# yshen47/SGAM_NeurIPS22

Hardware: AMD Instinct MI355X
Metric: generated RGB-D frames/sec (256x256, GoogleEarth) (higher is better)
Workload: dtype f32; 1 GPU; GoogleEarth-Infinite 256x256 inference loop (BASELINE configs[2]): forward-splat warp (N<=3) + VQGAN encode/quantise(4096)/decode + frame feedback, in-HBM frame store; frames_per_gpu=1105, scenes=1, parallelism=scene-parallel x1, launch=hip-graph replay of the VQGAN forward, f32_products=exact hi/lo fp16 split on the fp16 matrix cores, fp32 accumulate

## Files before the change

include/sgam_hip.h:

```cpp
#ifndef SGAM_HIP_H
#define SGAM_HIP_H

#include <stdint.h>

#ifdef __cplusplus
extern "C" {
#endif

#define SGAM_OK 0
#define SGAM_EINVAL (-1)
#define SGAM_EALIGN (-2)
#define SGAM_EWORKSPACE (-3)

int sgam_abi_version(void);
const char *sgam_build_info(void);
const char *sgam_build_commit(void);
const char *sgam_build_digest(void);

int sgam_prof_enable(int32_t on);
int sgam_prof_mark_empty(void *stream);
int32_t sgam_prof_count(void);
int sgam_prof_get(int32_t i, const char **kernel, const char **where, float *ms, double *flops, double *bytes);
int sgam_prof_get_shape(int32_t i, int32_t *mnks);

// ... 19 lines not shown
                            float *out, void *workspace, int64_t workspace_bytes, void *stream);

int sgam_pack_conv_weight(const float *w_oihw, float *w_packed, int32_t Cout, int32_t Cin, int32_t KH,
                          int32_t KW, int32_t Cout_pad, int32_t Cin_pad, void *stream);

int sgam_f32x_set_range_flag(int32_t *device_flag);
int64_t sgam_conv2d_f32x_workspace_bytes(const sgam_conv_desc *d);
int sgam_conv2d_f32x_plan(const sgam_conv_desc *d, int32_t *bm, int32_t *bn, int32_t *ksplit);
int sgam_conv2d_nhwc_f32x(const sgam_conv_desc *d, const float *x, float a_scale, const void *w_planes,
                          float w_scale, const float *bias, const float *residual, float *out, void *workspace,
                          int64_t workspace_bytes, void *stream);
int sgam_pack_conv_weight_f32x(const float *w_oihw, void *w_planes, float w_scale, int32_t Cout, int32_t Cin,
                               int32_t KH, int32_t KW, int32_t Cout_pad, int32_t Cin_pad, void *stream);
int32_t sgam_conv2d_f32x_stats_chunks(const sgam_conv_desc *d);
int32_t sgam_conv2d_f32x_stats_mode(const sgam_conv_desc *d);
int sgam_conv2d_stats_nhwc_f32x(const sgam_conv_desc *d, const float *x, float a_scale, const void *w_planes,
                                float w_scale, const float *bias, const float *residual, float *out,
                                double *gn_partial, void *workspace, int64_t workspace_bytes, void *stream);
int sgam_groupnorm_from_partials_f32(const float *x, const double *partial, int32_t nchunk, const float *gamma,
                                     const float *beta, float *y, int32_t B, int32_t HW, int32_t C, int32_t groups,
                                     float eps, int32_t fuse_swish, void *workspace, int64_t workspace_bytes, void *stream);
int32_t sgam_conv2d_f32x_gn_fusable(const sgam_conv_desc *d);
int32_t sgam_conv2d_f32x_uses_halo(const sgam_conv_desc *d);
int sgam_conv2d_gn_nhwc_f32x(const sgam_conv_desc *d, const float *x, const float *gn_mean_rstd, const float *gn_gamma,
                             const float *gn_beta, int32_t gn_swish, const void *w_planes, float w_scale, const float *bias,
                             const float *residual, float *out, double *gn_partial, void *workspace, int64_t workspace_bytes,
                             void *stream);
int32_t sgam_conv2d_f32x_gn_foldable(const sgam_conv_desc *d, int32_t chunks_in);
int sgam_conv2d_gnp_nhwc_f32x(const sgam_conv_desc *d, const float *x, const double *gn_partial_in, int32_t chunks_in, float eps,
                              const float *gn_gamma, const float *gn_beta, int32_t gn_swish, const void *w_planes, float w_scale,
                              const float *bias, const float *residual, float *out, double *gn_partial, void *workspace,
                              int64_t workspace_bytes, void *stream);
int sgam_groupnorm_stats_from_partials_f32(const double *partial, int32_t nchunk, float *mean_rstd, int32_t B, int32_t HW,
                                           int32_t C, int32_t groups, float eps, void *stream);
int sgam_groupnorm_meanrstd_nhwc_f32(const float *x, float *mean_rstd, int32_t B, int32_t HW, int32_t C, int32_t groups,
                                     float eps, void *workspace, int64_t workspace_bytes, void *stream);
int sgam_split_rows_f32x(const float *x, void *planes, float scale, int32_t N, int32_t K, int32_t ld, void *stream);

int64_t sgam_conv2d_h16_workspace_bytes(const sgam_conv_desc *d);
int sgam_conv2d_h16_plan(const sgam_conv_desc *d, int32_t *bm, int32_t *bn, int32_t *ksplit);
int sgam_conv2d_nhwc_h16(const sgam_conv_desc *d, int32_t ht, const void *x, const void *w_packed,
                         const float *bias, const void *residual, void *out, int32_t out_f32, void *workspace,
                         int64_t workspace_bytes, void *stream);
int32_t sgam_conv2d_h16_generic_stats_chunks(const sgam_conv_desc *d);
int sgam_conv2d_stats_nhwc_h16(const sgam_conv_desc *d, int32_t ht, const void *x, const void *w_packed, const float *bias,
                               const void *residual, void *out, int32_t out_f32, double *gn_partial, void *workspace,
// ... 295 lines not shown
```

sgam_neurips22_amd/_lib.py:

```python
import ctypes
import os

_PKG = os.path.dirname(os.path.abspath(__file__))
LIB_PATH = os.environ.get("SGAM_HIP_LIB") or os.path.join(_PKG, "lib", "libsgam_hip.so")

c_i32, c_i64, c_f32, c_vp = ctypes.c_int32, ctypes.c_int64, ctypes.c_float, ctypes.c_void_p


class ConvDesc(ctypes.Structure):
    _fields_ = [(n, c_i32) for n in (
        "B", "Hi", "Wi", "Cin", "Ho", "Wo", "N", "KH", "KW", "stride", "pad_t", "pad_l", "upsample2x",
        "lda", "ldb", "ldc", "ldr", "n_valid", "bias_per_row", "plan_bm", "plan_bn", "plan_ksplit")]


class TsdfGrid(ctypes.Structure):
    _fields_ = [("voxel_length", c_f32), ("sdf_trunc", c_f32), ("unit_base", c_i32 * 3), ("unit_dims", c_i32 * 3)]


class TsdfSrc(ctypes.Structure):
    _fields_ = [("depth", c_vp), ("rgb_u8", c_vp), ("cam2world", c_f32 * 16), ("world2cam", c_f32 * 16)]


class TsdfScene(ctypes.Structure):
    _fields_ = [("unit_table", c_vp), ("unit_stamp", c_vp), ("counters", c_vp), ("brick_list", c_vp), ("brick_tsdf", c_vp),
# ... 14 lines not shown
                              ctypes.POINTER(c_f32), ctypes.POINTER(ctypes.c_double), ctypes.POINTER(ctypes.c_double)]),
    "sgam_prof_get_shape": (c_i32, [c_i32, ctypes.POINTER(c_i32)]),
    "sgam_conv2d_workspace_bytes": (c_i64, [ctypes.POINTER(ConvDesc)]),
    "sgam_conv2d_plan": (c_i32, [ctypes.POINTER(ConvDesc), ctypes.POINTER(c_i32), ctypes.POINTER(c_i32),
                                 ctypes.POINTER(c_i32)]),
    "sgam_conv2d_nhwc_f32": (c_i32, [ctypes.POINTER(ConvDesc), c_vp, c_vp, c_vp, c_vp, c_vp, c_vp, c_i64, c_vp]),
    "sgam_conv2d_gn_nhwc_f32": (c_i32, [ctypes.POINTER(ConvDesc), c_vp, c_vp, c_i32, c_vp, c_vp, c_vp, c_vp, c_vp, c_i64,
                                        c_vp]),
    "sgam_pack_conv_weight": (c_i32, [c_vp, c_vp, c_i32, c_i32, c_i32, c_i32, c_i32, c_i32, c_vp]),
    "sgam_f32x_set_range_flag": (c_i32, [c_vp]),
    "sgam_conv2d_f32x_workspace_bytes": (c_i64, [ctypes.POINTER(ConvDesc)]),
    "sgam_conv2d_f32x_plan": (c_i32, [ctypes.POINTER(ConvDesc), ctypes.POINTER(c_i32), ctypes.POINTER(c_i32),
                                      ctypes.POINTER(c_i32)]),
    "sgam_conv2d_nhwc_f32x": (c_i32, [ctypes.POINTER(ConvDesc), c_vp, c_f32, c_vp, c_f32, c_vp, c_vp, c_vp, c_vp, c_i64,
                                      c_vp]),
    "sgam_conv2d_f32x_stats_chunks": (c_i32, [ctypes.POINTER(ConvDesc)]),
    "sgam_conv2d_f32x_stats_mode": (c_i32, [ctypes.POINTER(ConvDesc)]),
    "sgam_conv2d_stats_nhwc_f32x": (c_i32, [ctypes.POINTER(ConvDesc), c_vp, c_f32, c_vp, c_f32, c_vp, c_vp, c_vp, c_vp, c_vp,
                                            c_i64, c_vp]),
    "sgam_groupnorm_from_partials_f32": (c_i32, [c_vp, c_vp, c_i32, c_vp, c_vp, c_vp, c_i32, c_i32, c_i32, c_i32, c_f32,
                                                 c_i32, c_vp, c_i64, c_vp]),
    "sgam_conv2d_f32x_gn_fusable": (c_i32, [ctypes.POINTER(ConvDesc)]),
    "sgam_conv2d_f32x_uses_halo": (c_i32, [ctypes.POINTER(ConvDesc)]),
    "sgam_conv2d_gn_nhwc_f32x": (c_i32, [ctypes.POINTER(ConvDesc), c_vp, c_vp, c_vp, c_vp, c_i32, c_vp, c_f32, c_vp, c_vp,
                                         c_vp, c_vp, c_vp, c_i64, c_vp]),
    "sgam_conv2d_f32x_gn_foldable": (c_i32, [ctypes.POINTER(ConvDesc), c_i32]),
    "sgam_conv2d_gnp_nhwc_f32x": (c_i32, [ctypes.POINTER(ConvDesc), c_vp, c_vp, c_i32, c_f32, c_vp, c_vp, c_i32, c_vp, c_f32, c_vp,
                                          c_vp, c_vp, c_vp, c_vp, c_i64, c_vp]),
    "sgam_groupnorm_stats_from_partials_f32": (c_i32, [c_vp, c_i32, c_vp, c_i32, c_i32, c_i32, c_i32, c_f32, c_vp]),
    "sgam_groupnorm_meanrstd_nhwc_f32": (c_i32, [c_vp, c_vp, c_i32, c_i32, c_i32, c_i32, c_f32, c_vp, c_i64, c_vp]),
    "sgam_tsdf_integrate_srcs_f32": (c_i32, [ctypes.POINTER(TsdfGrid), ctypes.POINTER(TsdfSrc), c_i32, c_i32, c_i32, c_f32, c_f32, c_f32,
                                             c_f32, c_f32, c_i32, c_vp, c_vp, c_vp, c_vp, c_i32, c_vp, c_vp, c_i32, c_vp, c_vp, c_vp]),
    "sgam_tsdf_integrate_scenes_f32": (c_i32, [ctypes.POINTER(TsdfGrid), c_vp, c_vp, c_i32, c_i32, c_i32, c_i32, c_f32, c_f32, c_f32, c_f32,
                                               c_f32, c_i32, c_i32, c_vp, c_vp]),
    "sgam_tsdf_raycast_scenes_f32": (c_i32, [ctypes.POINTER(TsdfGrid), c_vp, c_vp, c_i32, c_i32, c_i32, c_f32, c_f32, c_f32, c_f32, c_f32,
                                             c_f32, c_vp, c_vp, c_vp]),
    "sgam_tsdf_ray_mult_f32": (c_i32, [c_i32, c_i32, c_f32, c_f32, c_f32, c_f32, c_vp, c_vp]),
    "sgam_tsdf_raycast_depth_f32": (c_i32, [ctypes.POINTER(TsdfGrid), c_i32, c_i32, c_f32, c_f32, c_f32, c_f32, c_vp, c_f32,
                                            c_f32, c_vp, c_vp, c_vp, c_vp, c_vp, c_vp]),
    "sgam_tsdf_extract_points_f32": (c_i32, [ctypes.POINTER(TsdfGrid), c_vp, c_vp, c_vp, c_vp, c_i64, c_vp, c_vp, c_vp, c_vp, c_vp]),
    "sgam_tsdf_mesh_workspace_bytes": (c_i64, [ctypes.POINTER(TsdfGrid), c_i32]),
    "sgam_tsdf_extract_mesh_f32": (c_i32, [ctypes.POINTER(TsdfGrid), c_vp, c_vp, c_vp, c_vp, c_i32, c_vp, c_i32, c_i32, c_f32, c_f32, c_f32,
                                           c_f32, c_f32, c_f32, c_vp, c_vp, c_vp, c_i64, c_vp, c_i64, c_vp, c_vp, c_i64, c_vp]),
    "sgam_mesh_render_depth_f32": (c_i32, [c_vp, c_i64, c_vp, c_i64, c_vp, c_i32, c_i32, c_f32, c_f32, c_f32, c_f32, c_vp, c_f32, c_f32,
                                           c_vp, c_vp]),
    "sgam_gemm_gn_f32x_fits": (c_i32, [c_i32, c_i32, c_i32, c_i32]),
# ... 183 lines not shown
```

sgam_neurips22_amd/csrc/conv_f32x.hip:

```cpp
#include <type_traits>

#include "sgam_common.h"

namespace {

constexpr int XGN_MAXC = 1024;

typedef unsigned int u32x4 __attribute__((ext_vector_type(4)));
typedef unsigned int u32x2 __attribute__((ext_vector_type(2)));
typedef _Float16 f16x8 __attribute__((ext_vector_type(8)));

struct XParams {
    const float *x, *bias, *res;
    const unsigned short *w;
    float *out, *ws;
    int B, Hi, Wi, Cin, Ho, Wo, N, KH, KW, stride, pad_t, pad_l, ups;
    int lda, ldb, ldc, ldr, n_valid, bias_per_row;
    int M, ksplit, iters_total, iters_per_split;
    int gx, gy, xcd_swizzle;
    unsigned x_bytes, w_plane_bytes;
    const float *gn_stats, *gn_gamma, *gn_beta;
    int gn_swish;
    const double *gn_partial_in;
    double gn_inv_n;
// ... 704 lines not shown
        if (s1 - s0 >= 2) {
            slab(s0, I2{}, I0{});
            slab(s0 + 1, I3{}, I3{});
        } else if (s0 < s1) {
            slab(s0, I3{}, I0{});
        }
    } else if (s0 < s1) {
        int sl = s0;
        for (; sl + 2 < s1; sl += 2) {
            slab(sl, I1{}, I0{});
            slab(sl + 1, I1{}, I3{});
        }
        slab(s1 - 2, I2{}, I0{});
        slab(s1 - 1, I3{}, I3{});
    }
    __syncthreads();

    xepilogue<BM, BN, WGM_>(p, acc, reinterpret_cast<float *>(smem), wave, lane, bx, bz, n0, [&](int row) {
        return (b * p.Ho + ty0 + (row >> TWS)) * p.Wo + tx0 + (row & (TW - 1));
    });
}


__global__ __launch_bounds__(256) void splitk_reduce_f32x_kernel(const XParams p) {
    const int64_t q = (int64_t)blockIdx.x * blockDim.x + threadIdx.x;
    const int nq = p.N / 4;
    const bool live = q < (int64_t)p.M * nq;
    const int m = live ? (int)(q / nq) : 0;
    const int n = live ? (int)(q - (int64_t)m * nq) * 4 : 0;
    float gs = 0.f, gss = 0.f;
    if (live) {
        const float *w0 = p.ws + (int64_t)m * p.N + n;
        const int64_t zs = (int64_t)p.M * p.N;
        float bv[4], rv[4];
#pragma unroll
        for (int e = 0; e < 4; ++e) {
            const bool ok = n + e < p.n_valid;
            bv[e] = (ok && p.bias) ? (p.bias_per_row ? p.bias[m] : p.bias[n + e]) : 0.f;
            rv[e] = (ok && p.res) ? p.res[(int64_t)m * p.ldr + n + e] : 0.f;
        }
        f32x4 s = *reinterpret_cast<const f32x4 *>(w0);
        int z = 1;
        for (; z + 4 <= p.ksplit; z += 4) {
            const f32x4 a = *reinterpret_cast<const f32x4 *>(w0 + z * zs), b = *reinterpret_cast<const f32x4 *>(w0 + (z + 1) * zs);
            const f32x4 c = *reinterpret_cast<const f32x4 *>(w0 + (z + 2) * zs), d = *reinterpret_cast<const f32x4 *>(w0 + (z + 3) * zs);
            s += a;
// ... 99 lines not shown
}

__device__ __forceinline__ int64_t frag_index(int64_t n, int64_t k, int64_t slabs_per_row) {
    const int64_t slab = k >> 5, kin = k & 31;
    const int64_t piece = (((kin >> 4) * 2) + ((kin >> 3) & 1)) * 32 + (n & 31);
    return (((n >> 5) * slabs_per_row + slab) * 256 + piece) * 8 + (kin & 7);
}

__global__ void pack_weight_f32x_kernel(const float *w, unsigned short *o, int Cout, int Cin, int KH, int KW, int Cout_pad,
                                        int Cin_pad, float scale) {
    const int64_t i = (int64_t)blockIdx.x * blockDim.x + threadIdx.x;
    const int taps = KH * KW;
    const int64_t total = (int64_t)Cout_pad * taps * Cin_pad;
    if (i >= total) return;
    const int c = (int)(i % Cin_pad);
    const int t = (int)((i / Cin_pad) % taps);
    const int n = (int)(i / ((int64_t)Cin_pad * taps));
    float v = 0.f;
    if (n < Cout && c < Cin) v = w[((int64_t)n * Cin + c) * taps + t] * scale;
    const _Float16 h = (_Float16)v;
    const _Float16 l = (_Float16)(v - (float)h);
    const int64_t k = (int64_t)t * Cin_pad + c;
    const int64_t q = frag_index(n, k, (int64_t)taps * Cin_pad / 32);
    o[q] = __builtin_bit_cast(unsigned short, h);
    o[q + 2 * 2 * 32 * 8] = __builtin_bit_cast(unsigned short, l);
}

__global__ void split_rows_f32x_kernel(const float *x, unsigned short *o, int N, int Np, int K, int Kp, int ld, float scale) {
    const int64_t i = (int64_t)blockIdx.x * blockDim.x + threadIdx.x;
    const int64_t total = (int64_t)Np * Kp;
    if (i >= total) return;
    const int n = (int)(i / Kp), k = (int)(i - (int64_t)n * Kp);
    const float v = (k < K && n < N) ? x[(int64_t)n * ld + k] * scale : 0.f;
    const _Float16 h = (_Float16)v;
    const _Float16 l = (_Float16)(v - (float)h);
    const int64_t q = frag_index(n, k, Kp / 32);
    o[q] = __builtin_bit_cast(unsigned short, h);
    o[q + 2 * 2 * 32 * 8] = __builtin_bit_cast(unsigned short, l);
}

struct XPlan {
    int bm, bn, ksplit, iters_total, iters_per_split;
};

static bool halo_shape(const sgam_conv_desc *d, int bm, int bn) {
    const bool tile_ok = (bm == 128 && bn == 128 && d->Wo % 16 == 0) || (bm == 64 && bn == 128 && d->Wo % 8 == 0) ||
// ... 30 lines not shown
    pl.iters_per_split = (pl.iters_total + ks - 1) / ks;
    if (halo_shape(d, pl.bm, pl.bn)) pl.iters_per_split = (pl.iters_per_split + 8) / 9 * 9;
    pl.ksplit = (pl.iters_total + pl.iters_per_split - 1) / pl.iters_per_split;
    return pl;
}

int xvalidate(const sgam_conv_desc *d) {
    if (!d) return SGAM_EINVAL;
    if (d->B <= 0 || d->Hi <= 0 || d->Wi <= 0 || d->Ho <= 0 || d->Wo <= 0 || d->N <= 0) return SGAM_EINVAL;
    if (d->Cin <= 0 || d->Cin % 8 != 0 || d->N % 4 != 0) return SGAM_EINVAL;
    if (d->KH <= 0 || d->KW <= 0 || d->stride <= 0) return SGAM_EINVAL;
    if (d->lda < d->Cin || d->lda % 4 != 0) return SGAM_EALIGN;
    if (d->ldb < d->KH * d->KW * d->Cin || d->ldb % 32 != 0) return SGAM_EALIGN;
    if (d->KH * d->KW > 1 && d->Cin % 32 != 0) return SGAM_EALIGN;
    if (d->n_valid <= 0 || d->n_valid > d->N || d->ldc < d->n_valid) return SGAM_EINVAL;
    if (d->n_valid % 4 != 0 || d->ldc % 4 != 0 || d->ldr % 4 != 0) return SGAM_EALIGN;
    if (d->plan_bm != 0 || d->plan_bn != 0) {
        const bool ok = (d->plan_bm == 128 && d->plan_bn == 128) || (d->plan_bm == 64 && d->plan_bn == 128) ||
                        (d->plan_bm == 128 && d->plan_bn == 32 && d->N == 32) ||
                        (d->plan_bm == 64 && d->plan_bn == 64);
        if (!ok || (d->plan_bn == 128 && d->N % 128 != 0)) return SGAM_EINVAL;
    }
    if (d->plan_ksplit < 0 || d->plan_ksplit > 64) return SGAM_EINVAL;
    return SGAM_OK;
}

}

extern "C" int64_t sgam_conv2d_f32x_workspace_bytes(const sgam_conv_desc *d) {
    if (xvalidate(d) != SGAM_OK) return -1;
    const XPlan pl = make_xplan(d);
    if (pl.ksplit <= 1) return 0;
    return (int64_t)pl.ksplit * d->B * d->Ho * d->Wo * d->N * (int64_t)sizeof(float);
}

extern "C" int sgam_conv2d_f32x_plan(const sgam_conv_desc *d, int32_t *bm, int32_t *bn, int32_t *ksplit) {
    const int rc = xvalidate(d);
    if (rc != SGAM_OK) return rc;
    const XPlan pl = make_xplan(d);
    if (bm) *bm = pl.bm;
    if (bn) *bn = pl.bn;
    if (ksplit) *ksplit = pl.ksplit;
    return SGAM_OK;
}

struct XExtra {
    const float *gn_stats = nullptr, *gn_gamma = nullptr, *gn_beta = nullptr;
    int gn_swish = 0;
    const double *gn_partial_in = nullptr;
    int gn_chunks_in = 0;
    float gn_eps = 1e-6f;
    double *gn_partial = nullptr;
};

static int conv_f32x_impl(const sgam_conv_desc *d, const float *x, float a_scale, const void *w_planes, float w_scale,
                          const float *bias, const float *residual, float *out, void *workspace, int64_t workspace_bytes,
                          void *stream, const XExtra &ex);

static bool halo_eligible(const sgam_conv_desc *d, const XPlan &pl, float a_scale) {
    return a_scale == 1.0f && halo_shape(d, pl.bm, pl.bn);
}

extern "C" int32_t sgam_conv2d_f32x_uses_halo(const sgam_conv_desc *d) {
    if (xvalidate(d) != SGAM_OK) return 0;
    return halo_eligible(d, make_xplan(d), 1.0f) ? 1 : 0;
}

extern "C" int32_t sgam_conv2d_f32x_gn_fusable(const sgam_conv_desc *d) {
    if (xvalidate(d) != SGAM_OK || d->upsample2x || d->Cin > XGN_MAXC) return 0;
    return halo_eligible(d, make_xplan(d), 1.0f) ? 1 : 0;
}

static int red_tc_for(const sgam_conv_desc *d) {
    const int hw = d->Ho * d->Wo, cpg = d->N / 32;
    if (d->N % 128 != 0 || d->n_valid != d->N || d->N > 1024) return 0;
    for (int tc = 32; tc >= 8; tc >>= 1) {
        const int tr = 1024 / tc;
        if (tc >= cpg && tc % cpg == 0 && (cpg & (cpg - 1)) == 0 && hw % tr == 0 && hw / tr <= 16) return tc;
    }
    return 0;
}

extern "C" int32_t sgam_conv2d_f32x_stats_chunks(const sgam_conv_desc *d) {
    if (xvalidate(d) != SGAM_OK) return -1;
    const XPlan pl = make_xplan(d);
    const int hw = d->Ho * d->Wo;
    if (d->N % 128 != 0 || d->n_valid != d->N) return 0;
    if (pl.ksplit == 1) {
// ... 92 lines not shown

    const int64_t xb = (((int64_t)d->B * d->Hi * d->Wi - 1) * d->lda + d->Cin) * 4;
    const int64_t wb = (int64_t)((d->N + 31) / 32 * 32) * d->ldb * 4;
    if (xb >= (1ll << 32) - 64 || wb >= (1ll << 32) - 256) return SGAM_EINVAL;
    p.x_bytes = (unsigned)xb; p.w_plane_bytes = (unsigned)wb;
    if (pl.ksplit > 1) {
        const int64_t need = (int64_t)pl.ksplit * p.M * p.N * (int64_t)sizeof(float);
        if (!workspace || workspace_bytes < need || !sgam_aligned16(workspace)) return SGAM_EWORKSPACE;
        p.ws = (float *)workspace;
    }
    p.gx = sgam_cdiv(p.M, pl.bm);
    p.gy = sgam_cdiv(p.N, pl.bn);
    p.xcd_swizzle = 1;
    const dim3 grid((unsigned)((int64_t)p.gx * p.gy * pl.ksplit));
    hipStream_t s = sgam_stream(stream);
#define XLAUNCH(BM_, BN_)                                                                                                   \
    do {                                                                                                                    \
        const dim3 blk(256 * wk_of(BM_, BN_));                                                                              \
        if (p.ups) SGAM_KLAUNCH((conv_gemm_f32x_kernel<BM_, BN_, true, false>), grid, blk, 0, s, p);                  \
        else if (a_scale != 1.0f) SGAM_KLAUNCH((conv_gemm_f32x_kernel<BM_, BN_, false, true>), grid, blk, 0, s, p);   \
        else SGAM_KLAUNCH((conv_gemm_f32x_kernel<BM_, BN_, false, false>), grid, blk, 0, s, p);                       \
    } while (0)
    if (p.ups && a_scale != 1.0f) return SGAM_EINVAL;
    if (d->KH * d->KW > 32) return SGAM_EINVAL;
    const bool halo = halo_eligible(d, pl, a_scale);
    const bool gn_tab_on = ex.gn_stats != nullptr;
    if ((gn_tab_on || ex.gn_partial_in) && !halo) return SGAM_EINVAL;
    if (gn_tab_on && d->Cin > XGN_MAXC) return SGAM_EINVAL;
    if (ex.gn_partial_in && (pl.bm != 64 || p.ups)) return SGAM_EINVAL;
    if (sgam_i_prof_on) sgam_i_prof_shape(p.M, d->n_valid, d->KH * d->KW * d->Cin, pl.ksplit);
    if (sgam_i_prof_on)
        sgam_i_prof_work(2.0 * p.M * d->n_valid * (double)(d->KH * d->KW * d->Cin),
                         4.0 * ((double)d->B * d->Hi * d->Wi * d->Cin + (double)d->n_valid * d->KH * d->KW * d->Cin +
                                (double)p.M * d->n_valid * (residual ? 2 : 1)));
    if (halo) {
        if (p.ups) {
            if (pl.bm == 128) SGAM_KLAUNCH((conv3x3_f32x_halo2_kernel<128, 128, false, true>), grid, dim3(256), 0, s, p);
            else SGAM_KLAUNCH((conv3x3_f32x_halo2_kernel<64, 128, false, true>), grid, dim3(256), 0, s, p);
        } else if (pl.bm == 128 && pl.bn == 32) {
            if (gn_tab_on) SGAM_KLAUNCH((conv3x3_f32x_halo2_kernel<128, 32, true>), grid, dim3(256), 0, s, p);
            else SGAM_KLAUNCH((conv3x3_f32x_halo2_kernel<128, 32, false>), grid, dim3(256), 0, s, p);
        } else if (pl.bm == 128) {
            if (gn_tab_on) SGAM_KLAUNCH((conv3x3_f32x_halo2_kernel<128, 128, true>), grid, dim3(256), 0, s, p);
            else SGAM_KLAUNCH((conv3x3_f32x_halo2_kernel<128, 128, false>), grid, dim3(256), 0, s, p);
        } else if (pl.bn == 64) {
            if (p.gn_partial_in) return SGAM_EINVAL;
            if (gn_tab_on) SGAM_KLAUNCH((conv3x3_f32x_halo2_kernel<64, 64, true>), grid, dim3(256), 0, s, p);
            else SGAM_KLAUNCH((conv3x3_f32x_halo2_kernel<64, 64, false>), grid, dim3(256), 0, s, p);
        } else {
            const int slabs_wg = p.iters_per_split / 9;
            const bool deep6 = (int64_t)grid.x * grid.y * grid.z <= 2 * 256 && p.iters_per_split % 9 == 0 &&
                               (p.gn_partial_in ? slabs_wg <= 2 : (slabs_wg % 2 == 0 && (p.iters_total / 9) % slabs_wg == 0));
            if (deep6 && p.gn_partial_in) SGAM_KLAUNCH((conv3x3_f32x_halo2_kernel<64, 128, true, false, true, 6>), grid, dim3(256), 0, s, p);
            else if (deep6 && gn_tab_on) SGAM_KLAUNCH((conv3x3_f32x_halo2_kernel<64, 128, true, false, false, 6>), grid, dim3(256), 0, s, p);
            else if (p.gn_partial_in) SGAM_KLAUNCH((conv3x3_f32x_halo2_kernel<64, 128, true, false, true>), grid, dim3(256), 0, s, p);
            else if (gn_tab_on) SGAM_KLAUNCH((conv3x3_f32x_halo2_kernel<64, 128, true>), grid, dim3(256), 0, s, p);
            else SGAM_KLAUNCH((conv3x3_f32x_halo2_kernel<64, 128, false>), grid, dim3(256), 0, s, p);
        }
    } else if (pl.bm == 128 && pl.bn == 128) XLAUNCH(128, 128);
// ... 3 lines not shown
    SGAM_LAUNCH_CHECK();
    if (pl.ksplit > 1) {
        const int64_t q = (int64_t)p.M * (p.N / 4);
        const int tc = p.gn_partial ? red_tc_for(d) : 0;
        if (tc == 32) SGAM_KLAUNCH(splitk_reduce_gm_f32x_kernel<32>, dim3((unsigned)(q / 256)), dim3(256), 0, s, p);
        else if (tc == 16) SGAM_KLAUNCH(splitk_reduce_gm_f32x_kernel<16>, dim3((unsigned)(q / 256)), dim3(256), 0, s, p);
        else if (tc == 8) SGAM_KLAUNCH(splitk_reduce_gm_f32x_kernel<8>, dim3((unsigned)(q / 256)), dim3(256), 0, s, p);
        else SGAM_KLAUNCH(splitk_reduce_f32x_kernel, dim3(sgam_cdiv(q, 256)), dim3(256), 0, s, p);
        SGAM_LAUNCH_CHECK();
    }
    return SGAM_OK;
}

extern "C" int sgam_pack_conv_weight_f32x(const float *w_oihw, void *w_planes, float w_scale, int32_t Cout, int32_t Cin,
                                          int32_t KH, int32_t KW, int32_t Cout_pad, int32_t Cin_pad, void *stream) {
    if (!w_oihw || !w_planes || Cout <= 0 || Cin <= 0 || KH <= 0 || KW <= 0 || Cout_pad < Cout || Cin_pad < Cin || Cin_pad % 32 || Cout_pad % 32) return SGAM_EINVAL;
    const int64_t total = (int64_t)Cout_pad * KH * KW * Cin_pad;
    SGAM_KLAUNCH(pack_weight_f32x_kernel, dim3(sgam_cdiv(total, 256)), dim3(256), 0, sgam_stream(stream), w_oihw,
                       (unsigned short *)w_planes, Cout, Cin, KH, KW, Cout_pad, Cin_pad, w_scale);
    SGAM_LAUNCH_CHECK();
    return SGAM_OK;
}

extern "C" int sgam_split_rows_f32x(const float *x, void *planes, float scale, int32_t N, int32_t K, int32_t ld, void *stream) {
    if (!x || !planes || N <= 0 || K <= 0 || ld < K) return SGAM_EINVAL;
    const int Kp = (K + 31) / 32 * 32, Np = (N + 31) / 32 * 32;
    const int64_t total = (int64_t)Np * Kp;
    SGAM_KLAUNCH(split_rows_f32x_kernel, dim3(sgam_cdiv(total, 256)), dim3(256), 0, sgam_stream(stream), x,
                       (unsigned short *)planes, N, Np, K, Kp, ld, scale);
    SGAM_LAUNCH_CHECK();
    return SGAM_OK;
}

extern "C" int sgam_debug_f32x_occupancy(int which) {
    int n = -1;
    hipError_t e;
    if (which == 0) e = hipOccupancyMaxActiveBlocksPerMultiprocessor(&n, conv_gemm_f32x_kernel<128, 128, false, false>, 256, 0);
    else if (which == 1) e = hipOccupancyMaxActiveBlocksPerMultiprocessor(&n, conv_gemm_f32x_kernel<64, 128, false, false>, 256, 0);
    else e = hipOccupancyMaxActiveBlocksPerMultiprocessor(&n, conv_gemm_f32x_kernel<64, 64, false, false>, 256 * wk_of(64, 64), 0);
    return e == hipSuccess ? n : -(int)e;
}
```

sgam_neurips22_amd/ops.py:

```python
import ctypes
import os

import torch

from . import _lib
from ._lib import ConvDesc, SgamHipError, check

from ._opscore import *
from ._opscore import _c, _dense_nhwc, _f32c, _need_cuda, _p, _set_gn_stats, _stats_buffer, _stream, _workspace


F32_MODE = os.environ.get("SGAM_F32_MODE", "split")
PANEL_GEMM = os.environ.get("SGAM_PANEL_GEMM", "1") == "1"
PANEL_MIN_WGS = int(os.environ.get("SGAM_PANEL_MIN_WGS", "1"))
FUSE_GN_STATS = os.environ.get("SGAM_FUSE_GN_STATS", "1") == "1"
FUSE_GN_APPLY = os.environ.get("SGAM_FUSE_GN_APPLY", "1") == "1"


_RANGE_FLAGS = {}
_RANGE_FLAG_ACTIVE = None


def _dev_index(device):
    d = torch.device(device)
# ... 17 lines not shown

RANGE_FLAG_EPOCH = 0


def f32x_range_tripped(reset=True, device=None):
    i = _RANGE_FLAG_ACTIVE if device is None else _dev_index(device)
    t = _RANGE_FLAGS.get(i)
    if t is None:
        return False
    hit = bool(t.item())
    if hit and reset:
        t.zero_()
    return hit


def set_f32_mode(mode):
    global F32_MODE
    if mode not in ("split", "mfma"):
        raise ValueError(mode)
    F32_MODE = mode


class SplitWeight:
    __slots__ = ("planes", "scale", "shape")

    def __init__(self, planes, scale, n=None, k=None):
        np_, kp = planes.shape[0] * 32, planes.shape[1] * 32
        self.planes, self.scale, self.shape = planes, scale, (np_ if n is None else n, kp if k is None else k)

    def stride(self, dim):
        return self.planes.shape[1] * 32 if dim == 0 else 1

    @property
    def dtype(self):
        return "f32x"

    @property
    def is_cuda(self):
        return self.planes.is_cuda


class FragWeightH16:
    __slots__ = ("planes", "shape")

    def __init__(self, planes):
        self.planes, self.shape = planes, (planes.shape[0] * 32, planes.shape[1] * 32)

    def stride(self, dim):
        return self.shape[1] if dim == 0 else 1

    @property
# ... 21 lines not shown

def split_rows(x2d, scale=1.0):
    _need_cuda(x2d)
    N, K = x2d.shape
    planes = torch.empty((round_up(N, 32) // 32, round_up(K, 32) // 32, 256, 8), device=x2d.device, dtype=torch.float16)
    check(_lib.load().sgam_split_rows_f32x(_p(x2d), _p(planes), float(scale), N, K, x2d.stride(0), _stream()),
          "sgam_split_rows_f32x")
    return SplitWeight(planes, float(scale), N, K)


def pack_conv_weight(w_oihw, cout_pad=None, cin_pad=None, dtype=torch.float32):
    _need_cuda(w_oihw)
    w = _f32c(w_oihw.detach())
    cout, cin, kh, kw = w.shape
    if cout_pad is None and dtype == "f32x" and kh * kw == 9 and cout <= 32:
        cout_pad = 32
    cout_pad = cout_pad or round_up(cout, 128 if ((dtype == "f32x" or dtype in H16) and kh * kw == 9) else 64)
    cin_pad = cin_pad or round_up(cin, 32)
    if dtype == "f32x":
        planes = torch.empty((cout_pad // 32, kh * kw * cin_pad // 32, 256, 8), device=w.device, dtype=torch.float16)
        scale = _pow2_scale(float(w.abs().max()))
        check(_lib.load().sgam_pack_conv_weight_f32x(_p(w), _p(planes), scale, cout, cin, kh, kw, cout_pad, cin_pad,
                                                     _stream()), "sgam_pack_conv_weight_f32x")
        return SplitWeight(planes, scale)
    out = torch.empty((cout_pad, kh * kw * cin_pad), device=w.device, dtype=dtype)
    if dtype == torch.float32:
        check(_lib.load().sgam_pack_conv_weight(_p(w), _p(out), cout, cin, kh, kw, cout_pad, cin_pad, _stream()),
              "sgam_pack_conv_weight")
    else:
        check(_lib.load().sgam_pack_conv_weight_h16(_p(w), _p(out), H16[dtype], cout, cin, kh, kw, cout_pad, cin_pad,
                                                    _stream()), "sgam_pack_conv_weight_h16")
    return out


PLAN_CACHE = {}
PLAN_RECORD = None
_PLAN_FILE = os.environ.get("SGAM_PLAN_FILE") or os.path.join(os.path.dirname(os.path.abspath(__file__)), "tuned_plans_gfx950.json")


def plan_key(desc, dtype):
    return (f"{str(dtype).replace('torch.', '')}|B{desc.B}|{desc.Hi}x{desc.Wi}x{desc.Cin}|{desc.Ho}x{desc.Wo}|N{desc.N}|"
            f"k{desc.KH}x{desc.KW}s{desc.stride}u{desc.upsample2x}")


def load_plans(path=_PLAN_FILE):
    PLAN_CACHE.clear()
    if os.path.exists(path) and not os.environ.get("SGAM_NO_TUNED_PLANS"):
        import json
        with open(path) as f:
            PLAN_CACHE.update({k: tuple(v) for k, v in json.load(f).get("plans", {}).items()})
    return len(PLAN_CACHE)


def _apply_plan(desc, dtype):
    if PLAN_RECORD is not None:
        PLAN_RECORD.setdefault(plan_key(desc, dtype), None)
    if desc.plan_bm == 0 and desc.plan_ksplit == 0:
        pl = PLAN_CACHE.get(plan_key(desc, dtype))
        if pl:
            desc.plan_bm, desc.plan_bn, desc.plan_ksplit = pl


def conv_plan(desc, h16=False, split=False):
    bm, bn, ks = ctypes.c_int32(), ctypes.c_int32(), ctypes.c_int32()
    lib = _lib.load()
    fn = lib.sgam_conv2d_f32x_plan if split else (lib.sgam_conv2d_h16_plan if h16 else lib.sgam_conv2d_plan)
    check(fn(ctypes.byref(desc), ctypes.byref(bm), ctypes.byref(bn), ctypes.byref(ks)), "sgam_conv2d_plan")
    return bm.value, bn.value, ks.value


ATTN_BLOCK_H16 = os.environ.get("SGAM_ATTN_BLOCK_H16", "1") != "0"
ATTN_BLOCK_H16_PROJ = os.environ.get("SGAM_ATTN_BLOCK_H16_PROJ", "1") != "0"
ATTN_BLOCK_F32X = os.environ.get("SGAM_ATTN_BLOCK_F32X", "1") != "0"
ATTN_SMALL = os.environ.get("SGAM_ATTN_SMALL", "1") != "0"


def _run_conv(desc, x, w, bias, residual, out, gn=None, a_scale=1.0, norm=None):
    lib = _lib.load()
    split = isinstance(w, SplitWeight)
    _apply_plan(desc, "f32x" if split else x.dtype)
    if norm is not None:
        gamma, beta, swish, groups, eps = norm
        d = ctypes.byref(desc)
        fusable = (split and FUSE_GN_APPLY and x.dtype == torch.float32 and x.dim() == 4 and groups == 32 and eps == 1e-6
                   and x.shape[3] % 128 == 0 and lib.sgam_conv2d_f32x_gn_fusable(d) == 1)
        st = gn_stats(x)
        h16_fusable = (x.dtype in H16 and FUSE_GN_APPLY and x.dim() == 4 and groups == 32 and eps == 1e-6
                       and x.shape[3] % 128 == 0 and x.shape[3] <= 1024 and not desc.upsample2x and _h16_frag(w, desc) is not None)
        if fusable and st is not None and lib.sgam_conv2d_f32x_gn_foldable(d, st[1]) == 1:
            gn = (st, gamma, beta, swish, eps)
        elif fusable and (st is not None or x.shape[1] * x.shape[2] > 1024):
            gn = (groupnorm_meanrstd(x, eps), gamma, beta, swish)
        elif h16_fusable and st is not None and lib.sgam_conv2d_h16_gn_foldable(d, st[1]) == 1:
            gn = (st, gamma, beta, swish, eps)
        elif h16_fusable:
            gn = (groupnorm_meanrstd(x, eps), gamma, beta, swish)
        else:
            x = groupnorm_nhwc(x, gamma, beta, swish, groups, eps)
    family = _conv_f32x if split else (_conv_h16 if x.dtype in H16 else _conv_f32)
    return _set_gn_stats(out, *family(lib, desc, x, w, bias, residual, out, gn, a_scale))


def _h16_frag(w, desc):
# ... 535 lines not shown
```

sgam_neurips22_amd/testing.py:

```python
import zlib

import numpy as np
import torch


def synthetic_state_dict(reference_state_dict, seed=0, codebook_sigma=1.0):
    out = {}
    for name in sorted(reference_state_dict.keys()):
        ref = reference_state_dict[name]
        shape = tuple(ref.shape) if hasattr(ref, "shape") else tuple(ref)
        g = torch.Generator().manual_seed((zlib.crc32(name.encode()) + 7919 * seed) % (2 ** 31))
        if name.endswith("embedding.weight"):
            t = torch.randn(shape, generator=g) * codebook_sigma
        elif ".norm" in name or name.startswith("norm") or "norm_out" in name:
            t = torch.randn(shape, generator=g) * 0.1
            if name.endswith("weight"):
                t = t + 1.0
        elif name.endswith("bias"):
            t = (torch.rand(shape, generator=g) * 2 - 1) * 0.1
        else:
            fan_in = int(np.prod(shape[1:])) if len(shape) > 1 else shape[0]
            b = (3.0 / fan_in) ** 0.5
            t = (torch.rand(shape, generator=g) * 2 - 1) * b
        out[name] = t.float()
# ... 269 lines not shown
        with open(os.path.join(root, f"{split}.txt"), "w") as fh:
            fh.write("\n".join(out[split]) + "\n")
    return out


def frame_list_dir(preferred):
    import atexit
    import os
    import shutil
    import tempfile
    preferred = os.path.abspath(str(preferred))
    if "im" not in preferred:
        os.makedirs(preferred, exist_ok=True)
        return preferred
    for base in (tempfile.gettempdir(), "/tmp", "/dev/shm"):
        if "im" in os.path.abspath(base) or not os.path.isdir(base):
            continue
        for _ in range(64):
            d = tempfile.mkdtemp(prefix="sgds", dir=base)
            atexit.register(shutil.rmtree, d, True)
            if "im" not in d:
                return d
    raise RuntimeError(f"no directory without 'im' in its path found for the single-frame datasets (tried beside {preferred})")
```

Baseline: 394.2 frames/s.

## Add sub-pixel phase decomposition for nearest-upsample 3x3 convs in f32x path

Adds a kernel that computes nearest-2x-upsample followed by a 3x3 conv as four 2x2 phase convolutions on the low-resolution input, using pre-summed phase weights (16 taps per channel instead of 36 effective). This removes the redundant MACs from convolving duplicated upsampled pixels and shrinks the halo loaded per tile. A new weight-packing routine builds the phase weights lazily and caches them, and Python dispatch switches eligible 128x128 halo-tile upsample convs to this path. The cost is extra weight memory, a more complex hand-scheduled kernel, and a different fp32 summation order for the combined weights.

```diff
diff --git a/include/sgam_hip.h b/include/sgam_hip.h
--- a/include/sgam_hip.h
+++ b/include/sgam_hip.h
@@ -65,6 +65,9 @@
                                      float eps, int32_t fuse_swish, void *workspace, int64_t workspace_bytes, void *stream);
 int32_t sgam_conv2d_f32x_gn_fusable(const sgam_conv_desc *d);
 int32_t sgam_conv2d_f32x_uses_halo(const sgam_conv_desc *d);
+int32_t sgam_conv2d_f32x_ups_phase(const sgam_conv_desc *d);
+int sgam_pack_conv_weight_f32x_ups_phase(const float *w_oihw, void *w_planes, float w_scale, int32_t Cout, int32_t Cin,
+                                         int32_t Cout_pad, int32_t Cin_pad, void *stream);
 int sgam_conv2d_gn_nhwc_f32x(const sgam_conv_desc *d, const float *x, const float *gn_mean_rstd, const float *gn_gamma,
                              const float *gn_beta, int32_t gn_swish, const void *w_planes, float w_scale, const float *bias,
                              const float *residual, float *out, double *gn_partial, void *workspace, int64_t workspace_bytes,
diff --git a/sgam_neurips22_amd/_lib.py b/sgam_neurips22_amd/_lib.py
--- a/sgam_neurips22_amd/_lib.py
+++ b/sgam_neurips22_amd/_lib.py
@@ -60,6 +60,8 @@
                                                  c_i32, c_vp, c_i64, c_vp]),
     "sgam_conv2d_f32x_gn_fusable": (c_i32, [ctypes.POINTER(ConvDesc)]),
     "sgam_conv2d_f32x_uses_halo": (c_i32, [ctypes.POINTER(ConvDesc)]),
+    "sgam_conv2d_f32x_ups_phase": (c_i32, [ctypes.POINTER(ConvDesc)]),
+    "sgam_pack_conv_weight_f32x_ups_phase": (c_i32, [c_vp, c_vp, c_f32, c_i32, c_i32, c_i32, c_i32, c_vp]),
     "sgam_conv2d_gn_nhwc_f32x": (c_i32, [ctypes.POINTER(ConvDesc), c_vp, c_vp, c_vp, c_vp, c_i32, c_vp, c_f32, c_vp, c_vp,
                                          c_vp, c_vp, c_vp, c_i64, c_vp]),
     "sgam_conv2d_f32x_gn_foldable": (c_i32, [ctypes.POINTER(ConvDesc), c_i32]),
diff --git a/sgam_neurips22_amd/csrc/conv_f32x.hip b/sgam_neurips22_amd/csrc/conv_f32x.hip
--- a/sgam_neurips22_amd/csrc/conv_f32x.hip
+++ b/sgam_neurips22_amd/csrc/conv_f32x.hip
@@ -750,6 +750,170 @@
 }
 
 
+__global__ __launch_bounds__(256, 2) void conv3x3_f32x_ups_phase_kernel(const XParams p) {
+    constexpr int BM = 128, BN = 128, TH = 8, TW = 16, NBR = 2;
+    constexpr int HROWS = TH / 2 + 2, HWID = TW / 2 + 2, HR = HROWS * HWID;
+    constexpr int XBK = 32, XLD = XBK + 8, LP = 448;
+    constexpr int HPL = HROWS * LP, HBUF = 2 * HPL;
+    constexpr int NH = (HR * 8 + 255) / 256;
+    constexpr int OP_BYTES = 2 * HBUF * 2;
+    constexpr int EPI_BYTES = 4 * BM * (32 + 4) * 4;
+    constexpr int SM_BYTES = OP_BYTES > EPI_BYTES ? OP_BYTES : EPI_BYTES;
+    __shared__ __attribute__((aligned(16))) unsigned short smem[SM_BYTES / 2];
+
+    const int tid = threadIdx.x;
+    const int lane = tid & 63;
+    const int wave = tid >> 6;
+    int bx, by, bz;
+    xcd_block(p, bx, by, bz);
+    const int n0 = by * BN;
+    const int tiles_x = p.Wo / TW, tiles_img = tiles_x * (p.Ho / TH);
+    const int b = bx / tiles_img;
+    const int t_img = bx - b * tiles_img;
+    const int ty0 = (t_img / tiles_x) * TH, tx0 = (t_img % tiles_x) * TW;
+
+    const __amdgpu_buffer_rsrc_t rx = __builtin_amdgcn_make_buffer_rsrc((void *)p.x, 0, (int)p.x_bytes, 0x00020000);
+    const __amdgpu_buffer_rsrc_t rw = __builtin_amdgcn_make_buffer_rsrc((void *)p.w, 0, (int)p.w_plane_bytes, 0x00020000);
+
+    const int s0 = (bz * p.iters_per_split) / 9, s1 = min(p.iters_total, (bz + 1) * p.iters_per_split) / 9;
+
+    unsigned h_off[NH];
+    int h_lds[NH];
+#pragma unroll
+    for (int j = 0; j < NH; ++j) {
+        const int idx = tid + 256 * j;
+        const int row = idx >> 3, col4 = idx & 7;
+        const int hy = row / HWID, hx = row - hy * HWID;
+        const int iy = ty0 / 2 + hy - 1, ix = tx0 / 2 + hx - 1;
+        const bool ok = row < HR && (unsigned)iy < (unsigned)p.Hi && (unsigned)ix < (unsigned)p.Wi;
+        h_off[j] = ok ? (unsigned)(((b * p.Hi + iy) * p.Wi + ix) * p.lda + col4 * 4) * 4u : 0xFFFFFFFFu;
+        h_lds[j] = row < HR ? hy * LP + hx * XLD + col4 * 4 : -1;
+    }
+    const unsigned bf_off = ((unsigned)((n0 + wave * 32) >> 5) * ((unsigned)p.ldb / 32u) * 256u + (unsigned)lane) * 16u;
+
+    f32x4 hreg[NH];
+    auto hload = [&](int ch, bool live) {
+        const unsigned coff = (unsigned)ch * (XBK * 4u);
+#pragma unroll
+        for (int j = 0; j < NH; ++j)
+            hreg[j] = __builtin_bit_cast(f32x4, __builtin_amdgcn_raw_buffer_load_b128(rx, (int)(live ? h_off[j] : 0xFFFFFFFFu), (int)coff, 0));
+    };
+    auto hprep_piece = [&](const int j) {
+        u32x2 hi, lo;
+        split4(hreg[j], hi, lo);
+        hreg[j] = __builtin_bit_cast(f32x4, u32x4{hi[0], hi[1], lo[0], lo[1]});
+    };
+    auto hstore = [&](int hbuf) {
+        unsigned short *halo = smem + hbuf * HBUF;
+#pragma unroll
+        for (int j = 0; j < NH; ++j) {
+            const u32x4 q = __builtin_bit_cast(u32x4, hreg[j]);
+            if (h_lds[j] >= 0) {
+                *reinterpret_cast<u32x2 *>(halo + h_lds[j]) = u32x2{q[0], q[1]};
+                *reinterpret_cast<u32x2 *>(halo + HPL + h_lds[j]) = u32x2{q[2], q[3]};
+            }
+        }
+    };
+
+    u32x4 bq[NBR][4][2];
+    auto bload = [&](const int set, const int q, int ch, bool live) {
+        const int kk = q >> 2, t = q & 3;
+        const unsigned vo = live ? bf_off : 0xFFFFFFF0u;
+#pragma unroll
+        for (int ph = 0; ph < 4; ++ph) {
+            const unsigned koff = (unsigned)((t * 4 + ph) * p.Cin + ch * XBK) * 128u;
+#pragma unroll
+            for (int pl = 0; pl < 2; ++pl)
+                bq[set][ph][pl] = __builtin_amdgcn_raw_buffer_load_b128(rw, (int)vo, (int)(koff + (unsigned)((pl * 2 + kk) * 1024)), 0);
+        }
+    };
+
+    f32x16 acc[4][1];
+#pragma unroll
+    for (int i = 0; i < 4; ++i)
+#pragma unroll
+        for (int e = 0; e < 16; ++e) acc[i][0][e] = 0.f;
+
+    const int frag_row = lane & 31;
+    const int a_base = (frag_row >> 3) * LP + (frag_row & 7) * XLD + (lane >> 5) * 8;
+
+    int hcur = 0;
+    hload(s0, s0 < s1);
+#pragma unroll
+    for (int q = 0; q < NBR - 1; ++q) bload(q, q, s0, s0 < s1);
+#pragma unroll
+    for (int j = 0; j < NH; ++j) hprep_piece(j);
+    hstore(0);
+    if (s0 + 1 < s1) hload(s0 + 1, true);
+    __syncthreads();
+
+    u32x4 fa[2][4][2];
+    unsigned a_lds = 0;
+    auto afrag = [&](const int set, const int q) {
+        const int kk = q >> 2, t = q & 3;
+        const int ns = t == 0 ? 4 : (t == 1 ? 1 : 2);
+#pragma unroll
+        for (int sl = 0; sl < ns; ++sl) {
+            const int dy = t == 0 ? 2 * (sl >> 1) - 1 : (t == 2 ? 2 * sl - 1 : 0);
+            const int dx = t == 0 ? 2 * (sl & 1) - 1 : (t == 3 ? 2 * sl - 1 : 0);
+            XDS_READ(fa[set][sl][0], a_lds, 2 * ((1 + dy) * LP + (1 + dx) * XLD + kk * 16));
+            XDS_READ(fa[set][sl][1], a_lds, 2 * ((1 + dy) * LP + (1 + dx) * XLD + kk * 16 + HPL));
+        }
+    };
+    auto await = [&](const int set, const int q) {
+        const int t = q & 3;
+        if (t == 0)
+            asm volatile("s_waitcnt lgkmcnt(2)" : "+v"(fa[set][0][0]), "+v"(fa[set][0][1]), "+v"(fa[set][1][0]), "+v"(fa[set][1][1]),
+                         "+v"(fa[set][2][0]), "+v"(fa[set][2][1]), "+v"(fa[set][3][0]), "+v"(fa[set][3][1]));
+        else if (t == 1)
+            asm volatile("s_waitcnt lgkmcnt(4)" : "+v"(fa[set][0][0]), "+v"(fa[set][0][1]));
+        else if (t == 2)
+            asm volatile("s_waitcnt lgkmcnt(4)" : "+v"(fa[set][0][0]), "+v"(fa[set][0][1]), "+v"(fa[set][1][0]), "+v"(fa[set][1][1]));
+        else if (q < 7)
+            asm volatile("s_waitcnt lgkmcnt(8)" : "+v"(fa[set][0][0]), "+v"(fa[set][0][1]), "+v"(fa[set][1][0]), "+v"(fa[set][1][1]));
+        else
+            asm volatile("s_waitcnt lgkmcnt(0)" : "+v"(fa[set][0][0]), "+v"(fa[set][0][1]), "+v"(fa[set][1][0]), "+v"(fa[set][1][1]));
+    };
+    auto slab = [&](const int sl) {
+        constexpr int RB = 0;
+        const bool has_next = sl + 1 < s1, has_next2 = sl + 2 < s1;
+        a_lds = (unsigned)(uintptr_t)(__attribute__((address_space(3))) const unsigned short *)(smem + hcur * HBUF) + 2u * (unsigned)a_base;
+#pragma unroll
+        for (int q = 0; q < 8; ++q) {
+            const int set = (q + RB) % NBR;
+            const int qq = q + NBR - 1;
+            if (qq < 8) bload((qq + RB) % NBR, qq, sl, true);
+            else bload((qq + RB) % NBR, qq - 8, sl + 1, has_next);
+            if (q >= 1 && q <= NH) hprep_piece(q - 1);
+            if (q == NH + 1) {
+                hstore(hcur ^ 1);
+                hload(sl + 2, has_next2);
+            }
+            if (q == 0) afrag(0, 0);
+            if (q < 7) afrag((q + 1) & 1, q + 1);
+            await(q & 1, q);
+            const int t = q & 3;
+#pragma unroll
+            for (int term = 0; term < 3; ++term)
+#pragma unroll
+                for (int ph = 0; ph < 4; ++ph) {
+                    const int slot = t == 0 ? ph : (t == 1 ? 0 : (t == 2 ? ph >> 1 : ph & 1));
+                    acc[ph][0] = mfma16(fa[q & 1][slot][term == 0 ? 1 : 0], bq[set][ph][term == 1 ? 1 : 0], acc[ph][0]);
+                }
+        }
+        __syncthreads();
+        hcur ^= 1;
+    };
+    for (int sl = s0; sl < s1; ++sl) slab(sl);
+    __syncthreads();
+
+    xepilogue<BM, BN, 1>(p, acc, reinterpret_cast<float *>(smem), wave, lane, bx, bz, n0, [&](int row) {
+        const int ph = row >> 5, i = (row >> 3) & 3, j = row & 7;
+        return (b * p.Ho + ty0 + 2 * i + (ph >> 1)) * p.Wo + tx0 + 2 * j + (ph & 1);
+    });
+}
+#undef XDS_READ
+
 __global__ __launch_bounds__(256) void splitk_reduce_f32x_kernel(const XParams p) {
     const int64_t q = (int64_t)blockIdx.x * blockDim.x + threadIdx.x;
     const int nq = p.N / 4;
@@ -895,6 +1059,32 @@
     const _Float16 l = (_Float16)(v - (float)h);
     const int64_t k = (int64_t)t * Cin_pad + c;
     const int64_t q = frag_index(n, k, (int64_t)taps * Cin_pad / 32);
+    o[q] = __builtin_bit_cast(unsigned short, h);
+    o[q + 2 * 2 * 32 * 8] = __builtin_bit_cast(unsigned short, l);
+}
+
+__global__ void pack_weight_f32x_ups_phase_kernel(const float *w, unsigned short *o, int Cout, int Cin, int Cout_pad, int Cin_pad,
+                                                  float scale) {
+    const int64_t i = (int64_t)blockIdx.x * blockDim.x + threadIdx.x;
+    const int64_t total = (int64_t)Cout_pad * 16 * Cin_pad;
+    if (i >= total) return;
+    const int c = (int)(i % Cin_pad);
+    const int u = (int)((i / Cin_pad) % 16);
+    const int n = (int)(i / ((int64_t)Cin_pad * 16));
+    const int t = u >> 2, a = (u >> 1) & 1, b = u & 1;
+    const int r = (t == 0 || t == 2) ? a : 1 - a, s = (t == 0 || t == 3) ? b : 1 - b;
+    const int ky0 = a == 0 ? r : 2 * r, ky1 = a == 0 ? 2 * r : 1 + r;
+    const int kx0 = b == 0 ? s : 2 * s, kx1 = b == 0 ? 2 * s : 1 + s;
+    float v = 0.f;
+    if (n < Cout && c < Cin) {
+        const float *wp = w + ((int64_t)n * Cin + c) * 9;
+        for (int ky = ky0; ky <= ky1; ++ky)
+            for (int kx = kx0; kx <= kx1; ++kx) v = (ky == ky0 && kx == kx0) ? wp[ky * 3 + kx] : v + wp[ky * 3 + kx];
+        v *= scale;
+    }
+    const _Float16 h = (_Float16)v;
+    const _Float16 l = (_Float16)(v - (float)h);
+    const int64_t q = frag_index(n, (int64_t)u * Cin_pad + c, (int64_t)16 * Cin_pad / 32);
     o[q] = __builtin_bit_cast(unsigned short, h);
     o[q + 2 * 2 * 32 * 8] = __builtin_bit_cast(unsigned short, l);
 }
@@ -971,6 +1161,7 @@
         if (!ok || (d->plan_bn == 128 && d->N % 128 != 0)) return SGAM_EINVAL;
     }
     if (d->plan_ksplit < 0 || d->plan_ksplit > 64) return SGAM_EINVAL;
+    if (d->upsample2x < 0 || d->upsample2x > 2) return SGAM_EINVAL;
     return SGAM_OK;
 }
 
@@ -1013,6 +1204,18 @@
 extern "C" int32_t sgam_conv2d_f32x_uses_halo(const sgam_conv_desc *d) {
     if (xvalidate(d) != SGAM_OK) return 0;
     return halo_eligible(d, make_xplan(d), 1.0f) ? 1 : 0;
+}
+
+static bool phase_shape(const sgam_conv_desc *d, const XPlan &pl) {
+    return d->upsample2x && pl.bm == 128 && pl.bn == 128 && halo_shape(d, 128, 128);
+}
+
+extern "C" int32_t sgam_conv2d_f32x_ups_phase(const sgam_conv_desc *d) {
+    if (xvalidate(d) != SGAM_OK || !d->upsample2x) return 0;
+    const XPlan pl = make_xplan(d);
+    if (!phase_shape(d, pl)) return 0;
+    if (d->upsample2x == 2) return d->ldb >= 16 * d->Cin ? 1 : 0;
+    return 0;
 }
 
 extern "C" int32_t sgam_conv2d_f32x_gn_fusable(const sgam_conv_desc *d) {
@@ -1151,6 +1354,8 @@
         else SGAM_KLAUNCH((conv_gemm_f32x_kernel<BM_, BN_, false, false>), grid, blk, 0, s, p);                       \
     } while (0)
     if (p.ups && a_scale != 1.0f) return SGAM_EINVAL;
+    const bool phase = d->upsample2x == 2;
+    if (phase && (!phase_shape(d, pl) || d->ldb < 16 * d->Cin || a_scale != 1.0f)) return SGAM_EINVAL;
     if (d->KH * d->KW > 32) return SGAM_EINVAL;
     const bool halo = halo_eligible(d, pl, a_scale);
     const bool gn_tab_on = ex.gn_stats != nullptr;
@@ -1163,7 +1368,8 @@
                          4.0 * ((double)d->B * d->Hi * d->Wi * d->Cin + (double)d->n_valid * d->KH * d->KW * d->Cin +
                                 (double)p.M * d->n_valid * (residual ? 2 : 1)));
     if (halo) {
-        if (p.ups) {
+        if (phase) SGAM_KLAUNCH(conv3x3_f32x_ups_phase_kernel, grid, dim3(256), 0, s, p);
+        else if (p.ups) {
             if (pl.bm == 128) SGAM_KLAUNCH((conv3x3_f32x_halo2_kernel<128, 128, false, true>), grid, dim3(256), 0, s, p);
             else SGAM_KLAUNCH((conv3x3_f32x_halo2_kernel<64, 128, false, true>), grid, dim3(256), 0, s, p);
         } else if (pl.bm == 128 && pl.bn == 32) {
@@ -1213,6 +1419,16 @@
     return SGAM_OK;
 }
 
+extern "C" int sgam_pack_conv_weight_f32x_ups_phase(const float *w_oihw, void *w_planes, float w_scale, int32_t Cout, int32_t Cin,
+                                                    int32_t Cout_pad, int32_t Cin_pad, void *stream) {
+    if (!w_oihw || !w_planes || Cout <= 0 || Cin <= 0 || Cout_pad < Cout || Cin_pad < Cin || Cin_pad % 32 || Cout_pad % 32) return SGAM_EINVAL;
+    const int64_t total = (int64_t)Cout_pad * 16 * Cin_pad;
+    SGAM_KLAUNCH(pack_weight_f32x_ups_phase_kernel, dim3(sgam_cdiv(total, 256)), dim3(256), 0, sgam_stream(stream), w_oihw,
+                       (unsigned short *)w_planes, Cout, Cin, Cout_pad, Cin_pad, w_scale);
+    SGAM_LAUNCH_CHECK();
+    return SGAM_OK;
+}
+
 extern "C" int sgam_split_rows_f32x(const float *x, void *planes, float scale, int32_t N, int32_t K, int32_t ld, void *stream) {
     if (!x || !planes || N <= 0 || K <= 0 || ld < K) return SGAM_EINVAL;
     const int Kp = (K + 31) / 32 * 32, Np = (N + 31) / 32 * 32;
diff --git a/sgam_neurips22_amd/ops.py b/sgam_neurips22_amd/ops.py
--- a/sgam_neurips22_amd/ops.py
+++ b/sgam_neurips22_amd/ops.py
@@ -63,11 +63,12 @@
 
 
 class SplitWeight:
-    __slots__ = ("planes", "scale", "shape")
-
-    def __init__(self, planes, scale, n=None, k=None):
+    __slots__ = ("planes", "scale", "shape", "src", "ups_phase")
+
+    def __init__(self, planes, scale, n=None, k=None, src=None):
         np_, kp = planes.shape[0] * 32, planes.shape[1] * 32
         self.planes, self.scale, self.shape = planes, scale, (np_ if n is None else n, kp if k is None else k)
+        self.src, self.ups_phase = src, None
 
     def stride(self, dim):
         return self.planes.shape[1] * 32 if dim == 0 else 1
@@ -135,7 +136,7 @@
         scale = _pow2_scale(float(w.abs().max()))
         check(_lib.load().sgam_pack_conv_weight_f32x(_p(w), _p(planes), scale, cout, cin, kh, kw, cout_pad, cin_pad,
                                                      _stream()), "sgam_pack_conv_weight_f32x")
-        return SplitWeight(planes, scale)
+        return SplitWeight(planes, scale, src=w if kh * kw == 9 else None)
     out = torch.empty((cout_pad, kh * kw * cin_pad), device=w.device, dtype=dtype)
     if dtype == torch.float32:
         check(_lib.load().sgam_pack_conv_weight(_p(w), _p(out), cout, cin, kh, kw, cout_pad, cin_pad, _stream()),
@@ -146,6 +147,19 @@
     return out
 
 
+def ups_phase_weight(sw):
+    if sw.ups_phase is None:
+        if sw.src is None:
+            raise SgamHipError("ups_phase_weight: not a 3x3 weight from pack_conv_weight(dtype='f32x')")
+        cout, cin = sw.src.shape[:2]
+        cout_pad, cin_pad = sw.planes.shape[0] * 32, sw.planes.shape[1] * 32 // 9
+        planes = torch.empty((cout_pad // 32, 16 * cin_pad // 32, 256, 8), device=sw.planes.device, dtype=torch.float16)
+        check(_lib.load().sgam_pack_conv_weight_f32x_ups_phase(_p(sw.src), _p(planes), sw.scale, cout, cin, cout_pad, cin_pad,
+                                                               _stream()), "sgam_pack_conv_weight_f32x_ups_phase")
+        sw.ups_phase = SplitWeight(planes, sw.scale)
+    return sw.ups_phase
+
+
 PLAN_CACHE = {}
 PLAN_RECORD = None
 _PLAN_FILE = os.environ.get("SGAM_PLAN_FILE") or os.path.join(os.path.dirname(os.path.abspath(__file__)), "tuned_plans_gfx950.json")
@@ -153,7 +167,7 @@
 
 def plan_key(desc, dtype):
     return (f"{str(dtype).replace('torch.', '')}|B{desc.B}|{desc.Hi}x{desc.Wi}x{desc.Cin}|{desc.Ho}x{desc.Wo}|N{desc.N}|"
-            f"k{desc.KH}x{desc.KW}s{desc.stride}u{desc.upsample2x}")
+            f"k{desc.KH}x{desc.KW}s{desc.stride}u{int(bool(desc.upsample2x))}")
 
 
 def load_plans(path=_PLAN_FILE):
@@ -171,7 +185,9 @@
     if desc.plan_bm == 0 and desc.plan_ksplit == 0:
         pl = PLAN_CACHE.get(plan_key(desc, dtype))
         if pl:
-            desc.plan_bm, desc.plan_bn, desc.plan_ksplit = pl
+            desc.plan_bm, desc.plan_bn, desc.plan_ksplit = pl[:3]
+            return pl[3] if len(pl) > 3 else 0
+    return 0
 
 
 def conv_plan(desc, h16=False, split=False):
@@ -191,7 +207,13 @@
 def _run_conv(desc, x, w, bias, residual, out, gn=None, a_scale=1.0, norm=None):
     lib = _lib.load()
     split = isinstance(w, SplitWeight)
-    _apply_plan(desc, "f32x" if split else x.dtype)
+    form = _apply_plan(desc, "f32x" if split else x.dtype)
+    if split and desc.upsample2x == 1 and w.src is not None and form != 1:
+        if form == 2 or lib.sgam_conv2d_f32x_ups_phase(ctypes.byref(desc)) == 1:
+            w = ups_phase_weight(w)
+            desc.upsample2x, desc.ldb = 2, w.stride(0)
+            if lib.sgam_conv2d_f32x_ups_phase(ctypes.byref(desc)) != 1:
+                raise SgamHipError(f"plan {plan_key(desc, 'f32x')}: the phase form needs the (128, 128) halo tile")
     if norm is not None:
         gamma, beta, swish, groups, eps = norm
         d = ctypes.byref(desc)
diff --git a/sgam_neurips22_amd/testing.py b/sgam_neurips22_amd/testing.py
--- a/sgam_neurips22_amd/testing.py
+++ b/sgam_neurips22_amd/testing.py
@@ -315,3 +315,22 @@
             if "im" not in d:
                 return d
     raise RuntimeError(f"no directory without 'im' in its path found for the single-frame datasets (tried beside {preferred})")
+
+
+def ups_phase_matrices(w):
+    import numpy as np
+    w = np.asarray(w)
+    mats, table = [], []
+    for u in range(16):
+        t, a, b = u >> 2, (u >> 1) & 1, u & 1
+        r = a if t in (0, 2) else 1 - a
+        s = b if t in (0, 3) else 1 - b
+        kys = ([0], [1, 2])[r] if a == 0 else ([0, 1], [2])[r]
+        kxs = ([0], [1, 2])[s] if b == 0 else ([0, 1], [2])[s]
+        m = None
+        for ky in kys:
+            for kx in kxs:
+                m = w[:, :, ky, kx].copy() if m is None else (m + w[:, :, ky, kx]).astype(w.dtype)
+        mats.append(m)
+        table.append((a, b, r, s))
+    return np.stack(mats), np.array(table)
```

New measurement: 394.7 frames/s, median of 4. Within noise of the previous version (+0.1%).
